# JanBeh/radiorust

Hardware: NVIDIA B200
Metric: complex MS/s via FreqShift->Filter->Downsampler (higher is better)
Workload: dtype f32

## Files before the change

radiorust_b200/csrc/rr_fused.cu:

```cuda
#include <cuda.h>
#include <cuda_runtime.h>

#include <algorithm>
#include <cstdio>
#include <cstdlib>
#include <mutex>

#include "rr_kernels.h"
#include "rr_poly.cuh"
#include "rr_pk.cuh"

namespace rr {

namespace {

constexpr int FK = 512;
constexpr int FRK = 10;
constexpr int T_WARPS = FRK / 2;
constexpr int T_THREADS = 32 * T_WARPS;
constexpr int F_ROWS = 32;
constexpr int PITCH = FRK * 8;
constexpr int STAGE_ROWS = 528;
constexpr int STAGE_BYTES = STAGE_ROWS * PITCH;
constexpr int TW_UNITS = 17;
constexpr int TW_BYTES = 16 * TW_UNITS * 16;
constexpr int YS_STRIDE = FK + 1;

constexpr int kFusedSlots = 6;
constexpr int kFusedSlotFloats = 2560;
__constant__ float4 c_fcoef[kFusedSlots * kFusedSlotFloats / 4];

__device__ __forceinline__ uint32_t s_u32(const void* p) { return (uint32_t)__cvta_generic_to_shared(p); }
__device__ __forceinline__ void mb_init(uint32_t bar, uint32_t count) {
    asm volatile("mbarrier.init.shared::cta.b64 [%0], %1;" ::"r"(bar), "r"(count) : "memory");
}
__device__ __forceinline__ void mb_expect_tx(uint32_t bar, uint32_t bytes) {
    asm volatile("mbarrier.arrive.expect_tx.shared::cta.b64 _, [%0], %1;" ::"r"(bar), "r"(bytes) : "memory");
}
__device__ __forceinline__ void mb_arrive(uint32_t bar) {
    asm volatile("mbarrier.arrive.release.cta.shared::cta.b64 _, [%0];" ::"r"(bar) : "memory");
}
__device__ __forceinline__ void mb_wait(uint32_t bar, uint32_t parity) {
    asm volatile(
        "{\n"
        ".reg .pred p;\n"
        "FWAIT_%=:\n"
        "mbarrier.try_wait.parity.acquire.cta.shared::cta.b64 p, [%0], %1;\n"
        "@p bra FDONE_%=;\n"
        "bra FWAIT_%=;\n"
        "FDONE_%=:\n"
        "}\n" ::"r"(bar),
        "r"(parity)
        : "memory");
}
__device__ __forceinline__ void mb_wait_long(uint32_t bar, uint32_t parity) {
    asm volatile(
        "{\n"
        ".reg .pred p;\n"
        "LWAIT_%=:\n"
        "mbarrier.try_wait.parity.acquire.cta.shared::cta.b64 p, [%0], %1, %2;\n"
        "@p bra LDONE_%=;\n"
        "bra LWAIT_%=;\n"
        "LDONE_%=:\n"
        "}\n" ::"r"(bar),
        "r"(parity), "r"(20000u)
        : "memory");
}
__device__ __forceinline__ pc f_lds(uint32_t addr) {
    pc r;
    asm volatile("ld.shared.v2.f32 {%0, %1}, [%2];" : "=f"(r.x), "=f"(r.y) : "r"(addr));
    return r;
}
__device__ __forceinline__ void f_lds2(uint32_t addr, pc& a, pc& b) {
    asm volatile("ld.shared.v4.f32 {%0, %1, %2, %3}, [%4];" : "=f"(a.x), "=f"(a.y), "=f"(b.x), "=f"(b.y) : "r"(addr));
}
__device__ __forceinline__ void f_sts(uint32_t addr, pc a) {
    asm volatile("st.shared.v2.f32 [%0], {%1, %2};" ::"r"(addr), "f"(a.x), "f"(a.y) : "memory");
}
__device__ __forceinline__ void f_sts2(uint32_t addr, pc a, pc b) {
    asm volatile("st.shared.v4.f32 [%0], {%1, %2, %3, %4};" ::"r"(addr), "f"(a.x), "f"(a.y), "f"(b.x), "f"(b.y) : "memory");
}
__device__ __forceinline__ void f_ldg2(const float4* p, pc& a, pc& b) {
    asm volatile("ld.global.nc.v4.f32 {%0, %1, %2, %3}, [%4];" : "=f"(a.x), "=f"(a.y), "=f"(b.x), "=f"(b.y) : "l"(p));
}

__device__ __forceinline__ pc f_rotation(uint32_t d, uint32_t numer_abs, uint32_t denom, double inv_m, int sign) {
    const uint32_t r = mulmod_fast(numer_abs, d % denom, denom, inv_m);
    double s, c;
    sincospi(2.0 * (double)r / (double)denom, &s, &c);
    return pc((float)c, (float)(sign < 0 ? -s : s));
}

__device__ __forceinline__ void f_pass1_store(pc (&v)[32], uint32_t tw_row, uint32_t xch_wr) {
    pdft_regs<32, +1>(v);
    pc w[3][2];
    f_lds2(tw_row, w[0][0], w[0][1]);
    f_lds2(tw_row + 16, w[1][0], w[1][1]);
#pragma unroll
    for (int m = 0; m < 16; ++m) {
        if (m + 2 < 16) f_lds2(tw_row + (m + 2) * 16, w[(m + 2) % 3][0], w[(m + 2) % 3][1]);
        f_sts(xch_wr + (2 * m) * PITCH, pcmul(v[2 * m], w[m % 3][0]));
        f_sts(xch_wr + (2 * m + 1) * PITCH, pcmul(v[2 * m + 1], w[m % 3][1]));
    }
}

#ifdef RR_FUSED_PROF
#define PROF(...) __VA_ARGS__
__device__ long long g_fused_prof[256 * 16];
#else
#define PROF(...)
#endif

struct FusedGeom {
    int steps, S0, hp, slot_bytes, slot_stride;
};
__host__ __device__ inline FusedGeom fused_geom(int P) {
    FusedGeom g;
    g.steps = P / 2;
    g.S0 = (g.steps + 1) / 2;
    g.hp = 2 * g.S0 + ((g.S0 & 1) ? 0 : 2);
    if (g.hp > P) g.hp = P;
    g.slot_bytes = F_ROWS * g.hp * 8;
    g.slot_stride = (g.slot_bytes + 127) / 128 * 128;
    return g;
}

template <int S_LO, int S_HI, bool HAS_NCO>
__device__ __forceinline__ void f_steps(pc (&acc)[FRK], const float4* __restrict__ xrow, const float4* __restrict__ crow, const float4* cf_base) {
#pragma unroll
    for (int st = S_LO; st < S_HI; ++st) {
        const float4 xv = xrow[st];
        pc x0(xv.x, xv.y), x1(xv.z, xv.w);
        if (HAS_NCO) {
            const float4 cv = crow[st];
            x0 = pcmul(x0, pc(cv.x, cv.y));
            x1 = pcmul(x1, pc(cv.z, cv.w));
        }
        const float4* cf = cf_base + st * 5;
        const float4 a0 = cf[0], a1 = cf[1], a2 = cf[2], a3 = cf[3], a4 = cf[4];
        const float k0[FRK] = {a0.x, a0.y, a0.z, a0.w, a1.x, a1.y, a1.z, a1.w, a2.x, a2.y};
        const float k1[FRK] = {a2.z, a2.w, a3.x, a3.y, a3.z, a3.w, a4.x, a4.y, a4.z, a4.w};
#pragma unroll
        for (int c = 0; c < FRK; ++c) {
            acc[c] = pfma_s(x0, k0[c], acc[c]);
            acc[c] = pfma_s(x1, k1[c], acc[c]);
        }
    }
}

}

template <int FW, int D, int NB, bool HAS_NCO, int PT>
__global__ void __launch_bounds__(T_THREADS + 32 * FW, 1)
k_fused(const __grid_constant__ CUtensorMap tmap, const FusedArgs a, const int n_streams) {
    extern __shared__ __align__(128) unsigned char smem[];
    const int warp = __shfl_sync(0xffffffffu, (int)(threadIdx.x >> 5), 0), lane = threadIdx.x & 31;
    const int P = PT > 0 ? PT : a.P;
    const FusedGeom geo = fused_geom(P);
    const int Lmax = a.Lmax, V = a.V, n_out = a.n_out;
    const int B = (n_out + V - 1) / V;
    const int n_tiles = (B * V + F_ROWS - 1) / F_ROWS;

    const int keep_bytes = ((Lmax * PITCH) + 127) / 128 * 128;
    unsigned char* const p_stage = smem;
    unsigned char* const p_tw = p_stage + 2 * STAGE_BYTES;
    unsigned char* const p_keep = p_tw + TW_BYTES;
    unsigned char* const p_ys = p_keep + keep_bytes;
    unsigned char* const p_ring = p_ys + (((size_t)NB * YS_STRIDE * 8 + 127) / 128 * 128);
    unsigned char* const p_colph = p_ring + (size_t)FW * D * geo.slot_stride;
    unsigned char* const p_bar = p_colph + (((size_t)FW * P * 8 + 127) / 128 * 128);
    const uint32_t bar_full = s_u32(p_bar), bar_empty = bar_full + 16, bar_ring = bar_full + 32;
    const uint32_t left_cnt = bar_ring + FW * D * 8;

    for (int e = threadIdx.x; e < 2 * STAGE_BYTES / 16; e += blockDim.x) reinterpret_cast<float4*>(p_stage)[e] = make_float4(0.f, 0.f, 0.f, 0.f);
    {
        const float2* __restrict__ twK = reinterpret_cast<const float2*>(a.twK);
        for (int e = threadIdx.x; e < FK; e += blockDim.x) {
            const int tr = e >> 5, k1 = e & 31;
            const float2 w = twK[(tr * k1) & (FK - 1)];
            const int off = (tr * TW_UNITS + (k1 >> 1)) * 16 + (k1 & 1) * 8;
            *reinterpret_cast<float2*>(p_tw + off) = w;
        }
    }
    if (threadIdx.x == 0) {
        asm volatile("prefetch.tensormap [%0];" ::"l"(&tmap) : "memory");
        mb_init(bar_full, FW);
        mb_init(bar_full + 8, FW);
        mb_init(bar_empty, T_WARPS);
        mb_init(bar_empty + 8, T_WARPS);
        for (int q = 0; q < FW * D; ++q) mb_init(bar_ring + q * 8, 1);
        asm volatile("st.shared.v2.u32 [%0], {%1, %1};" ::"r"(left_cnt), "r"(0u) : "memory");
        asm volatile("fence.mbarrier_init.release.cluster;" ::: "memory");
    }
    __syncthreads();

    const int n_my = (n_streams - (int)blockIdx.x + (int)gridDim.x - 1) / (int)gridDim.x;
    if (n_my <= 0) return;

    if (warp >= T_WARPS) {
        const int fw = warp - T_WARPS;
        const uint32_t ring_s = s_u32(p_ring) + fw * (D * geo.slot_stride);
        const uint32_t rbar = bar_ring + fw * (D * 8);
        float2* const colph = reinterpret_cast<float2*>(p_colph) + fw * P;
        const int steps = geo.steps, S0 = geo.S0, hp = geo.hp;
        const int half1_col0 = P - hp;
        const int J0 = (int)a.J0;
        const int hist_len = (int)(2 * a.n);
        const int hist_from = (int)a.hist_from;
        const int n_live = (n_out + F_ROWS - 1) / F_ROWS;
        const int rot_step = n_live % FW;
        auto tiles_from = [&](int j0) { return j0 < n_tiles ? (n_tiles - j0 + FW - 1) / FW : 0; };
        const int BV = B * V;
        const int tile_step = FW * F_ROWS;

        int i_so = 0, i_k = 0, i_half = 0, i_slot = 0;
        int i_j0 = fw, i_rot = 0, i_tw = tiles_from(fw);
        auto issue_next = [&]() {
            while (i_so < n_my) {
                if (i_k >= i_tw) {
                    ++i_so;
                    i_k = 0;
                    i_rot += rot_step;
                    if (i_rot >= FW) i_rot -= FW;
                    i_j0 = fw - i_rot + (fw < i_rot ? FW : 0);
                    i_tw = tiles_from(i_j0);
                    continue;
                }
                const int j = i_j0 + i_k * FW, half = i_half, so = i_so;
                i_half ^= 1;
                if (i_half == 0) ++i_k;
                const int rows_ok = min(F_ROWS, n_out - j * F_ROWS);
                if (rows_ok <= 0) continue;
                const int pos0 = j * (F_ROWS * P) - J0;
                const int coff = half ? half1_col0 : 0;
                const int sh = pos0 < 0 ? -1 : F_ROWS - rows_ok;
                if (lane == 0) {
                    mb_expect_tx(rbar + i_slot * 8, (uint32_t)geo.slot_bytes);
                    asm volatile("cp.async.bulk.tensor.3d.shared::cluster.global.mbarrier::complete_tx::bytes [%0], [%1, {%3, %4, %5}], [%2];" ::"r"(
                                     ring_s + i_slot * geo.slot_stride),
                                 "l"(&tmap), "r"(rbar + i_slot * 8), "r"(pos0 + coff - sh * P), "r"(sh), "r"((int)blockIdx.x + so * (int)gridDim.x)
                                 : "memory");
                }
                i_slot = (i_slot + 1 == D) ? 0 : i_slot + 1;
                return;
            }
        };
#pragma unroll 1
        for (int q = 0; q < D; ++q) issue_next();

        PROF(long long pr[8] = {0, 0, 0, 0, 0, 0, 0, 0}; const long long pr_t0 = clock64();)
        int c_slot = 0;
        uint32_t c_phase = 0;
        int gb_acq = -1;
        int gb_arr = -1;
        auto arrive_upto = [&](int gb_done) {
            for (int g2 = gb_arr + 1; g2 <= gb_done; ++g2) {
                while (gb_acq < g2) {
                    ++gb_acq;
                    mb_wait(bar_empty + (uint32_t)(gb_acq & 1) * 8, (uint32_t)(((gb_acq >> 1) & 1) ^ 1));
                }
                __syncwarp();
                if (lane == 0) mb_arrive(bar_full + (uint32_t)(g2 & 1) * 8);
            }
            if (gb_done > gb_arr) gb_arr = gb_done;
        };

        int rot = 0;
#pragma unroll 1
        for (int so = 0; so < n_my; ++so) {
            PROF(const long long pst0 = clock64();)
            const int s = (int)blockIdx.x + so * (int)gridDim.x;
            const int gb0 = so * B;
            const int j0 = fw - rot + (fw < rot ? FW : 0);
            const int tiles_w = tiles_from(j0);
            rot += rot_step;
            if (rot >= FW) rot -= FW;
            uint32_t denom = 1, numer_abs = 0, idx0 = 0;
            int sign = 0;
            float start = 0.f;
            pc rot_tile(1.f, 0.f);
            double inv_denom = 1.0;
            if (HAS_NCO && j0 < n_live) {
                const NcoStream ns = a.nco[s];
                denom = ns.denom;
                numer_abs = ns.numer_abs;
                sign = ns.sign;
                idx0 = ns.idx;
                start = (float)ns.start_phase;
                inv_denom = 1.0 / (double)denom;
                rot_tile = f_rotation((uint32_t)(tile_step * P), numer_abs, denom, inv_denom, sign);
                __syncwarp();
                for (int p = lane; p < P; p += 32) {
                    const pc c = f_rotation((uint32_t)p, numer_abs, denom, inv_denom, sign);
                    colph[p] = make_float2(c.x, c.y);
                }
                __syncwarp();
            }
            const float2* __restrict__ in = reinterpret_cast<const float2*>(a.in) + (long long)s * a.in_stride;
            const float2* __restrict__ hist_end = reinterpret_cast<const float2*>(a.hist2) + ((long long)s + 1) * hist_len;
            float2* __restrict__ hist_o = a.hist_out ? reinterpret_cast<float2*>(a.hist_out) + (long long)s * a.hist_stride : nullptr;
            float4* __restrict__ keep_o = reinterpret_cast<float4*>(reinterpret_cast<float2*>(a.ukeep_out) + (long long)s * a.ukeep_out_stride);
            const float4* cf_base = c_fcoef + a.coef_off4;
            const float4* __restrict__ crow = reinterpret_cast<const float4*>(colph);

            PROF(pr[7] += clock64() - pst0;)
            int blk = (j0 * F_ROWS) / V, off = (j0 * F_ROWS) - blk * V;
            pc rowph(1.f, 0.f);
#pragma unroll 1
            for (int k = 0; k < tiles_w; ++k) {
                const int r0 = (j0 + k * FW) * F_ROWS;
                const int row = r0 + lane;
                const int pos0 = r0 * P - J0;
                pc acc[FRK];
#pragma unroll
                for (int c = 0; c < FRK; ++c) acc[c] = pc(0.f, 0.f);
                PROF(long long pc0 = clock64();)
                if (r0 < n_out) {
                    if (HAS_NCO) {
                        if ((k & 15) == 0) {
                            const long long v = (long long)idx0 + pos0 + (long long)lane * P;
                            long long kk = v - (long long)floor((double)v * inv_denom) * (long long)denom;
                            if (kk < 0) kk += denom;
                            else if (kk >= (long long)denom) kk -= denom;
                            const cx<float> c = nco_phasor<float>(mulmod_fast(numer_abs, (uint32_t)kk, denom, inv_denom), denom, sign, start);
                            rowph = pc(c.x, c.y);
                        } else {
                            rowph = pcmul(rowph, rot_tile);
                        }
                    }
                    const int prow = pos0 + lane * P;
                    const bool to_hist = hist_o != nullptr && pos0 + F_ROWS * P > hist_from;
#pragma unroll 1
                    for (int half = 0; half < 2; ++half) {
                        const uint32_t slot_s = ring_s + c_slot * geo.slot_stride;
                        PROF(long long pw0 = clock64(); pr[0] += pw0 - pc0;)
                        mb_wait(rbar + c_slot * 8, c_phase);
                        PROF(long long pw1 = clock64(); pr[1] += pw1 - pw0;)
                        const int col0 = half ? half1_col0 : 0;
                        if (pos0 < 0) {
                            float2* dst = reinterpret_cast<float2*>(smem + (slot_s - s_u32(smem)));
                            const float r0x = __shfl_sync(0xffffffffu, rowph.x, 0), r0y = __shfl_sync(0xffffffffu, rowph.y, 0);
                            for (int cc = lane; cc < hp; cc += 32) {
                                const int p = col0 + cc;
                                const int pos = pos0 + p;
                                float2 q = make_float2(0.f, 0.f);
                                if (pos >= 0) {
                                    if (pos < (int)a.len) q = __ldg(in + pos);
                                } else if (pos >= -hist_len) {
                                    q = __ldg(hist_end + pos);
                                    if (HAS_NCO) {
                                        const float2 cph = colph[p];
                                        const pc y = pcmulc(pc(q.x, q.y), pcmul(pc(r0x, r0y), pc(cph.x, cph.y)));
                                        q = make_float2(y.x, y.y);
                                    }
                                }
                                dst[cc] = q;
                            }
                            __syncwarp();
                        }
                        const float4* __restrict__ xrow = reinterpret_cast<const float4*>(smem + (slot_s - s_u32(smem)) + lane * (hp * 8) - col0 * 8);
                        if (to_hist) {
                            const int st_lo = half ? S0 : 0, st_hi = half ? steps : S0;
#pragma unroll 2
                            for (int st = st_lo; st < st_hi; ++st) {
                                const float4 xv = xrow[st];
                                pc x0(xv.x, xv.y), x1(xv.z, xv.w);
                                if (HAS_NCO) {
                                    const float4 cv = crow[st];
                                    x0 = pcmul(x0, pc(cv.x, cv.y));
                                    x1 = pcmul(x1, pc(cv.z, cv.w));
                                }
                                const pc y0 = HAS_NCO ? pcmul(x0, rowph) : x0, y1 = HAS_NCO ? pcmul(x1, rowph) : x1;
                                const int jh = prow + 2 * st - hist_from;
                                if (row < n_out && jh >= -1) {
                                    if (jh >= 0) hist_o[jh] = make_float2(y0.x, y0.y);
                                    hist_o[jh + 1] = make_float2(y1.x, y1.y);
                                }
                                const float4* cf = cf_base + st * 5;
                                const float4 a0 = cf[0], a1 = cf[1], a2 = cf[2], a3 = cf[3], a4 = cf[4];
                                const float k0[FRK] = {a0.x, a0.y, a0.z, a0.w, a1.x, a1.y, a1.z, a1.w, a2.x, a2.y};
                                const float k1[FRK] = {a2.z, a2.w, a3.x, a3.y, a3.z, a3.w, a4.x, a4.y, a4.z, a4.w};
#pragma unroll
                                for (int c = 0; c < FRK; ++c) {
                                    acc[c] = pfma_s(x0, k0[c], acc[c]);
                                    acc[c] = pfma_s(x1, k1[c], acc[c]);
                                }
                            }
                        } else if constexpr (PT > 0) {
                            constexpr int STEPS_C = PT / 2, S0_C = (STEPS_C + 1) / 2;
                            if (half == 0) f_steps<0, S0_C, HAS_NCO>(acc, xrow, crow, cf_base);
                            else f_steps<S0_C, STEPS_C, HAS_NCO>(acc, xrow, crow, cf_base);
                        } else {
                            const int st_lo = half ? S0 : 0, st_hi = half ? steps : S0;
#pragma unroll 4
                            for (int st = st_lo; st < st_hi; ++st) {
                                const float4 xv = xrow[st];
                                pc x0(xv.x, xv.y), x1(xv.z, xv.w);
                                if (HAS_NCO) {
                                    const float4 cv = crow[st];
                                    x0 = pcmul(x0, pc(cv.x, cv.y));
                                    x1 = pcmul(x1, pc(cv.z, cv.w));
                                }
                                const float4* cf = cf_base + st * 5;
                                const float4 a0 = cf[0], a1 = cf[1], a2 = cf[2], a3 = cf[3], a4 = cf[4];
                                const float k0[FRK] = {a0.x, a0.y, a0.z, a0.w, a1.x, a1.y, a1.z, a1.w, a2.x, a2.y};
                                const float k1[FRK] = {a2.z, a2.w, a3.x, a3.y, a3.z, a3.w, a4.x, a4.y, a4.z, a4.w};
#pragma unroll
                                for (int c = 0; c < FRK; ++c) {
                                    acc[c] = pfma_s(x0, k0[c], acc[c]);
                                    acc[c] = pfma_s(x1, k1[c], acc[c]);
                                }
                            }
                        }
                        PROF(long long ps1 = clock64(); pr[2] += ps1 - pw1;)
                        asm volatile("fence.proxy.async.shared::cta;" ::: "memory");
                        __syncwarp();
                        PROF(long long ps2 = clock64(); pr[3] += ps2 - ps1;)
                        if (++c_slot == D) {
                            c_slot = 0;
                            c_phase ^= 1u;
                        }
                        issue_next();
                        PROF(pc0 = clock64(); pr[4] += pc0 - ps2;)
                    }
                }
                {
                    const int last_off = min(off + F_ROWS, BV - blk * V) - 1;
                    const int gb_hi = gb0 + blk + (last_off >= V ? 1 : 0);
                    PROF(long long pe0 = clock64(); pr[0] += pe0 - pc0;)
                    while (gb_acq < gb_hi) {
                        ++gb_acq;
                        mb_wait(bar_empty + (uint32_t)(gb_acq & 1) * 8, (uint32_t)(((gb_acq >> 1) & 1) ^ 1));
                    }
                    PROF(pc0 = clock64(); pr[5] += pc0 - pe0;)
                }
                if (row < BV) {
                    int b = blk, o = off + lane;
                    if (o >= V) {
                        o -= V;
                        ++b;
                    }
                    const uint32_t dst = s_u32(p_stage) + (uint32_t)((gb0 + b) & 1) * STAGE_BYTES + (Lmax + o) * PITCH;
                    const bool live = row < n_out;
                    const bool keep = live && row >= n_out - Lmax;
#pragma unroll
                    for (int c = 0; c < FRK; c += 2) {
                        pc y0 = acc[c], y1 = acc[c + 1];
                        if (HAS_NCO) {
                            y0 = pcmul(y0, rowph);
                            y1 = pcmul(y1, rowph);
                        }
                        if (!live) {
                            y0 = pc(0.f, 0.f);
                            y1 = pc(0.f, 0.f);
                        }
                        f_sts2(dst + c * 8, y0, y1);
                        if (keep) keep_o[((row - (n_out - Lmax)) * FRK + c) / 2] = make_float4(y0.x, y0.y, y1.x, y1.y);
                    }
                }
                __syncwarp();
                off += tile_step;
                while (off >= V) {
                    off -= V;
                    ++blk;
                }
                arrive_upto((k + 1 < tiles_w) ? gb0 + min(blk, B) - 1 : gb0 + B - 1);
                PROF(pr[6] += clock64() - pc0;)
            }
            if (tiles_w == 0) arrive_upto(gb0 + B - 1);
        }
        PROF(if (fw == 0 && lane == 0) {
            for (int q = 0; q < 7; ++q) g_fused_prof[blockIdx.x * 16 + q] = pr[q];
            g_fused_prof[blockIdx.x * 16 + 7] = pr[7];
            g_fused_prof[blockIdx.x * 16 + 8] = clock64() - pr_t0;
        })
        return;
    }

    const int tid = threadIdx.x;
    const int t = lane >> 1, gg = lane & 1;
    const int g = 2 * warp + gg;
    auto sync_t = [&]() { asm volatile("bar.sync 1, %0;" ::"n"(T_THREADS) : "memory"); };
    const uint32_t stage0 = s_u32(p_stage);
    const uint32_t tw_row = s_u32(p_tw) + t * (TW_UNITS * 16);
    const uint32_t tile_rd = t * PITCH + g * 8;
    const uint32_t xch_wr = 33 * t * PITCH + g * 8;
    const uint32_t xch_rd = t * PITCH + g * 8;
    const uint32_t keep_s = s_u32(p_keep) + warp * 16;
    float2* const ysave = reinterpret_cast<float2*>(p_ys);
    const float4* __restrict__ gtab = reinterpret_cast<const float4*>(a.gtab);
    const int hist_rows_per_lane = (Lmax + 31) / 32;

    const int n_blocks_total = n_my * B;
    auto copy_kept = [&](int so_k, int gb_k) {
        const uint32_t bytes = (uint32_t)(Lmax * PITCH), bar = bar_full + (uint32_t)(gb_k & 1) * 8;
        const float2* src = reinterpret_cast<const float2*>(a.ukeep_in) + (long long)((int)blockIdx.x + so_k * (int)gridDim.x) * a.ukeep_in_stride;
        asm volatile("fence.proxy.async.shared::cta;" ::: "memory");
        asm volatile("mbarrier.expect_tx.relaxed.cta.shared::cta.b64 [%0], %1;" ::"r"(bar), "r"(bytes) : "memory");
        asm volatile("cp.async.bulk.shared::cluster.global.mbarrier::complete_tx::bytes [%0], [%1], %2, [%3];" ::"r"(stage0 + (uint32_t)(gb_k & 1) * STAGE_BYTES),
                     "l"(src), "r"(bytes), "r"(bar)
                     : "memory");
    };
    if (tid == 0) {
        copy_kept(0, 0);
        if (B == 1 && n_my > 1) copy_kept(1, 1);
    }
    int parked = 0;
    int gb_first = 0;
    int so = 0, b = -1;
    PROF(long long tp[6] = {0, 0, 0, 0, 0, 0}; long long tc = clock64();)

#pragma unroll 1
    for (int gb = 0; gb < n_blocks_total; ++gb) {
        if (++b == B) {
            b = 0;
            ++so;
        }
        const int s = (int)blockIdx.x + so * (int)gridDim.x;
        const uint32_t stg = stage0 + (uint32_t)(gb & 1) * STAGE_BYTES;

        PROF({ long long n_ = clock64(); tp[0] += n_ - tc; tc = n_; })
        mb_wait_long(bar_full + (uint32_t)(gb & 1) * 8, (uint32_t)((gb >> 1) & 1));
        PROF({ long long n_ = clock64(); tp[1] += n_ - tc; tc = n_; })
#pragma unroll
        for (int q = 0; q < 12; ++q) {
            const int r = lane + 32 * q;
            if (q < hist_rows_per_lane && r < Lmax) {
                float4 nx;
                asm volatile("ld.shared.v4.f32 {%0, %1, %2, %3}, [%4];" : "=f"(nx.x), "=f"(nx.y), "=f"(nx.z), "=f"(nx.w) : "r"(stg + (V + r) * PITCH + warp * 16));
                if (b != 0) {
                    float4 h;
                    asm volatile("ld.shared.v4.f32 {%0, %1, %2, %3}, [%4];" : "=f"(h.x), "=f"(h.y), "=f"(h.z), "=f"(h.w) : "r"(keep_s + r * PITCH));
                    asm volatile("st.shared.v4.f32 [%0], {%1, %2, %3, %4};" ::"r"(stg + r * PITCH + warp * 16), "f"(h.x), "f"(h.y), "f"(h.z), "f"(h.w) : "memory");
                }
                asm volatile("st.shared.v4.f32 [%0], {%1, %2, %3, %4};" ::"r"(keep_s + r * PITCH), "f"(nx.x), "f"(nx.y), "f"(nx.z), "f"(nx.w) : "memory");
            }
        }
        if (b == 0 && n_out < Lmax) {
            float4* __restrict__ kout = reinterpret_cast<float4*>(reinterpret_cast<float2*>(a.ukeep_out) + (long long)s * a.ukeep_out_stride);
#pragma unroll 1
            for (int r = n_out + lane; r < Lmax; r += 32) {
                float4 h;
                asm volatile("ld.shared.v4.f32 {%0, %1, %2, %3}, [%4];" : "=f"(h.x), "=f"(h.y), "=f"(h.z), "=f"(h.w) : "r"(stg + r * PITCH + warp * 16));
                kout[((long long)(r - n_out) * FRK) / 2 + warp] = h;
            }
        }
        if (lane == 0) asm volatile("st.shared.v4.f32 [%0], {%1, %1, %1, %1};" ::"r"(stg + (FK - 1) * PITCH + warp * 16), "f"(0.f) : "memory");
        __syncwarp();

        pc acc[32];
        {
            pc v[32];
            const uint32_t src = stg + tile_rd;
#pragma unroll
            for (int m = 0; m < 32; ++m) v[m] = f_lds(src + m * (16 * PITCH));
            __syncwarp();
            f_pass1_store(v, tw_row, stg + xch_wr);
        }
        {
            const float4* gp = gtab + tid;
            pc h[16];
#pragma unroll
            for (int jj = 0; jj < 8; ++jj) f_ldg2(gp + jj * T_THREADS, h[2 * jj], h[2 * jj + 1]);
            __syncwarp();
#pragma unroll
            for (int which = 0; which < 2; ++which) {
                pc x[16];
#pragma unroll
                for (int tr = 0; tr < 16; ++tr) x[tr] = f_lds(stg + xch_rd + (33 * tr + 16 * which) * PITCH);
                pdft_regs<16, +1>(x);
#pragma unroll
                for (int k = 0; k < 16; ++k) acc[which * 16 + k] = pcmul(x[k], h[k]);
                if (which == 0) {
#pragma unroll
                    for (int jj = 0; jj < 8; ++jj) f_ldg2(gp + (8 + jj) * T_THREADS, h[2 * jj], h[2 * jj + 1]);
                }
            }
        }
        PROF({ long long n_ = clock64(); tp[2] += n_ - tc; tc = n_; })
        __syncwarp();
#pragma unroll
        for (int j = 0; j < 32; ++j) f_sts(stg + xch_rd + (16 * j) * PITCH, acc[j]);
        sync_t();
        if (parked == 0) gb_first = gb;
        {
            float2* ys = ysave + parked * YS_STRIDE;
            for (int o = tid; o < FK; o += T_THREADS) {
                const uint32_t src = stg + o * PITCH;
                pc sum(0.f, 0.f);
#pragma unroll
                for (int w = 0; w < T_WARPS; ++w) {
                    pc u0, u1;
                    f_lds2(src + w * 16, u0, u1);
                    sum = sum + u0;
                    sum = sum + u1;
                }
                const int j = o >> 4, tt = o & 15;
                ys[tt + 16 * (j >> 4) + 32 * (j & 15)] = make_float2(sum.x, sum.y);
            }
        }
        ++parked;
        PROF({ long long n_ = clock64(); tp[3] += n_ - tc; tc = n_; })

        if (parked == NB || gb + 1 == n_blocks_total) {
            sync_t();
#pragma unroll 1
            for (int j0 = 0; j0 < parked; j0 += FRK) {
                if (j0 + 2 * warp >= parked) continue;
                const int job = j0 + g;
                const bool active = job < parked;
                pc v[32];
                const float2* ys = ysave + (active ? job : 0) * YS_STRIDE;
#pragma unroll
                for (int i1 = 0; i1 < 32; ++i1) {
                    const float2 q = ys[t + 16 * i1];
                    v[i1] = active ? pc(q.x, -q.y) : pc(0.f, 0.f);
                }
                f_pass1_store(v, tw_row, stg + xch_wr);
                __syncwarp();
                const int gj = gb_first + (active ? job : 0);
                const int so_j = gj / B, b_j = gj - so_j * B;
                const int s_j = (int)blockIdx.x + so_j * (int)gridDim.x;
                float2* __restrict__ out = reinterpret_cast<float2*>(a.out) + (long long)s_j * a.out_stride;
                float2* __restrict__ out2 = a.out2 ? reinterpret_cast<float2*>(a.out2) + (long long)s_j * a.out2_stride : nullptr;
#pragma unroll
                for (int which = 0; which < 2; ++which) {
                    pc x[16];
#pragma unroll
                    for (int tr = 0; tr < 16; ++tr) x[tr] = f_lds(stg + xch_rd + (33 * tr + 16 * which) * PITCH);
                    pdft_regs<16, +1>(x);
                    if (active) {
#pragma unroll
                        for (int k2 = 0; k2 < 16; ++k2) {
                            const int i = t + 16 * which + 32 * k2;
                            if (i >= Lmax && i < Lmax + V) {
                                const long long o = (long long)b_j * V + (i - Lmax);
                                if (o < n_out) {
                                    float2* dst = (out2 != nullptr && o >= a.out_split) ? out2 + (o - a.out_split) : out + o;
                                    *dst = make_float2(x[k2].x, -x[k2].y);
                                }
                            }
                        }
                    }
                }
                __syncwarp();
            }
            parked = 0;
            sync_t();
        }
        PROF({ long long n_ = clock64(); tp[4] += n_ - tc; tc = n_; })
        __syncwarp();
        if (lane == 0) {
            uint32_t left;
            asm volatile("atom.acq_rel.cta.shared::cta.add.u32 %0, [%1], 1;" : "=r"(left) : "r"(left_cnt + (uint32_t)(gb & 1) * 4) : "memory");
            if (left % T_WARPS == T_WARPS - 1) {
                int b2 = b + 2, so2 = so;
                while (b2 >= B) {
                    b2 -= B;
                    ++so2;
                }
                if (b2 == 0 && so2 < n_my) copy_kept(so2, gb + 2);
            }
            mb_arrive(bar_empty + (uint32_t)(gb & 1) * 8);
        }
    }
    PROF(if (tid == 0) for (int q = 0; q < 5; ++q) g_fused_prof[blockIdx.x * 16 + 9 + q] = tp[q];)
}

namespace {

using EncodeFn = CUresult (*)(CUtensorMap*, CUtensorMapDataType, cuuint32_t, void*, const cuuint64_t*, const cuuint64_t*, const cuuint32_t*,
                              const cuuint32_t*, CUtensorMapInterleave, CUtensorMapSwizzle, CUtensorMapL2promotion, CUtensorMapFloatOOBfill);
EncodeFn fused_encode_fn() {
    static EncodeFn fn = nullptr;
    static std::once_flag once;
    std::call_once(once, [] {
        void* p = nullptr;
        cudaDriverEntryPointQueryResult q;
        if (cudaGetDriverEntryPoint("cuTensorMapEncodeTiled", &p, cudaEnableDefault, &q) == cudaSuccess && q == cudaDriverEntryPointSuccess)
            fn = reinterpret_cast<EncodeFn>(p);
    });
    return fn;
}

template <int FW, int D, int NB> size_t fused_smem(int P, int Lmax) {
    const FusedGeom geo = fused_geom(P);
    size_t b = 2 * (size_t)STAGE_BYTES + TW_BYTES;
    b += ((size_t)Lmax * PITCH + 127) / 128 * 128;
    b += ((size_t)NB * YS_STRIDE * 8 + 127) / 128 * 128;
    b += (size_t)FW * D * geo.slot_stride;
    b += ((size_t)FW * P * 8 + 127) / 128 * 128;
    b += 32 + (size_t)FW * D * 8 + 64;
    return b;
}

template <int FW, int D, int NB>
cudaError_t launch_cfg(int n_streams, const FusedArgs& a, const CUtensorMap& tm, int sm_count, cudaStream_t st) {
    const size_t smem = fused_smem<FW, D, NB>(a.P, a.Lmax);
    if (smem > (size_t)227 * 1024) return cudaErrorInvalidConfiguration;
    const int grid = std::min(n_streams, sm_count);
    void (*kern)(const CUtensorMap, const FusedArgs, const int);
    switch (a.P) {
        case 50: kern = a.nco ? k_fused<FW, D, NB, true, 50> : k_fused<FW, D, NB, false, 50>; break;
        case 40: kern = a.nco ? k_fused<FW, D, NB, true, 40> : k_fused<FW, D, NB, false, 40>; break;
        case 20: kern = a.nco ? k_fused<FW, D, NB, true, 20> : k_fused<FW, D, NB, false, 20>; break;
        default: return cudaErrorNotSupported;
    }
    const cudaError_t e = cudaFuncSetAttribute(kern, cudaFuncAttributeMaxDynamicSharedMemorySize, (int)smem);
    if (e != cudaSuccess) return e;
    kern<<<grid, T_THREADS + 32 * FW, smem, st>>>(tm, a, n_streams);
#ifdef RR_FUSED_PROF
    static int calls = 0;
    static int at = std::getenv("RR_FUSED_PROF_CALL") ? std::atoi(std::getenv("RR_FUSED_PROF_CALL")) : 12;
    if (++calls == at) {
        cudaDeviceSynchronize();
        long long h[256 * 16];
        cudaMemcpyFromSymbol(h, g_fused_prof, sizeof h);
        for (int c : {0, 100})
            fprintf(stderr,
                    "cta %d n_out %d F0: tile-head %lld ring-wait %lld steps %lld fence+sync %lld issue %lld empty-wait %lld finalize %lld stream-setup %lld | total %lld"
                    " || T0: pre %lld wait-full %lld fwd+prod %lld sum+park %lld inverse %lld\n",
                    c, a.n_out, h[c * 16], h[c * 16 + 1], h[c * 16 + 2], h[c * 16 + 3], h[c * 16 + 4], h[c * 16 + 5], h[c * 16 + 6], h[c * 16 + 7], h[c * 16 + 8], h[c * 16 + 9],
                    h[c * 16 + 10], h[c * 16 + 11], h[c * 16 + 12], h[c * 16 + 13]);
    }
#endif
    return cudaGetLastError();
}

}

int fused_coef_slots() { return kFusedSlots; }

bool fused_supported(int rank_pad, long long P, int Lmax) {
    if (rank_pad != FRK || !(P == 50 || P == 40 || P == 20) || fused_encode_fn() == nullptr) return false;
    if (Lmax < 1 || FK - 1 - Lmax < 128 || Lmax > 383) return false;
    if ((P / 2) * 2 * FRK > kFusedSlotFloats) return false;
    return fused_smem<7, 2, 5>((int)P, Lmax) <= (size_t)227 * 1024;
}

cudaError_t fused_upload_coef(int slot, const float* acoef, int P, cudaStream_t st) {
    if (slot < 0 || slot >= kFusedSlots) return cudaErrorInvalidValue;
    const size_t n = (size_t)(P / 2) * 2 * FRK;
    if (n > (size_t)kFusedSlotFloats) return cudaErrorInvalidValue;
    return cudaMemcpyToSymbolAsync(c_fcoef, acoef, n * sizeof(float), (size_t)slot * kFusedSlotFloats * sizeof(float), cudaMemcpyHostToDevice, st);
}

cudaError_t launch_fused(int n_streams, const FusedArgs& a0, int sm_count, cudaStream_t st) {
    EncodeFn enc = fused_encode_fn();
    if (!enc) return cudaErrorNotSupported;
    FusedArgs a = a0;
    a.coef_off4 = a.coef_slot * (kFusedSlotFloats / 4);
    if ((uintptr_t)a.ukeep_in % 16 != 0 || (n_streams > 1 && a.ukeep_in_stride % 2 != 0)) return cudaErrorInvalidValue;
    const FusedGeom geo = fused_geom(a.P);
    CUtensorMap tm;
    const cuuint64_t dims[3] = {(cuuint64_t)a.len, (cuuint64_t)F_ROWS, (cuuint64_t)n_streams};
    const cuuint64_t sstride = n_streams > 1 ? (cuuint64_t)a.in_stride * 8 : (((cuuint64_t)a.len * 8 + 15) / 16) * 16;
    const cuuint64_t strides[2] = {(cuuint64_t)a.P * 8, sstride};
    const cuuint32_t box[3] = {(cuuint32_t)geo.hp, (cuuint32_t)F_ROWS, 1};
    const cuuint32_t estr[3] = {1, 1, 1};
    const CUresult r = enc(&tm, CU_TENSOR_MAP_DATA_TYPE_UINT64, 3, const_cast<void*>(a.in), dims, strides, box, estr, CU_TENSOR_MAP_INTERLEAVE_NONE,
                           CU_TENSOR_MAP_SWIZZLE_NONE, CU_TENSOR_MAP_L2_PROMOTION_L2_128B, CU_TENSOR_MAP_FLOAT_OOB_FILL_NONE);
    if (r != CUDA_SUCCESS) return cudaErrorInvalidValue;
    static int cfg = -1;
    if (cfg < 0) {
        cfg = 0;
        if (const char* e = std::getenv("RR_FUSED_CFG")) cfg = std::atoi(e);
    }
    switch (cfg) {
        case 1: return launch_cfg<6, 2, 8>(n_streams, a, tm, sm_count, st);
        default: return launch_cfg<7, 2, 5>(n_streams, a, tm, sm_count, st);
    }
}

}
```

Measured before the change: 529,900.

## Process multiple row groups per filter warp with K column boxes

Generalizes the filter warps so each lane handles R rows (R=2 by default for long outputs), sharing coefficient and column-phasor loads across rows. Each input tile is also split into K column boxes (4 by default) rather than two halves, which keeps ring slots small while tiles get taller. The tensor map is now built per configuration, and the code falls back to R=1, K=2 for short outputs or when shared memory would overflow. The goal is to amortize coefficient loads and per-tile overhead over more rows, at the cost of higher register pressure (20 accumulators per lane) and more barrier and TMA round trips per tile.

Measured after the change: 419,000, median of 6. 20.9% lower.

```diff
diff --git a/radiorust_b200/csrc/rr_fused.cu b/radiorust_b200/csrc/rr_fused.cu
--- a/radiorust_b200/csrc/rr_fused.cu
+++ b/radiorust_b200/csrc/rr_fused.cu
@@ -112,54 +112,68 @@
 #endif
 
 struct FusedGeom {
-    int steps, S0, hp, slot_bytes, slot_stride;
+    int rows, steps, SB, hp, slot_bytes, slot_stride;
 };
-__host__ __device__ inline FusedGeom fused_geom(int P) {
-    FusedGeom g;
+__host__ __device__ constexpr FusedGeom fused_geom(int P, int R, int K) {
+    FusedGeom g{};
+    g.rows = F_ROWS * R;
     g.steps = P / 2;
-    g.S0 = (g.steps + 1) / 2;
-    g.hp = 2 * g.S0 + ((g.S0 & 1) ? 0 : 2);
+    g.SB = (g.steps + K - 1) / K;
+    g.hp = 2 * g.SB + ((g.SB & 1) ? 0 : 2);
     if (g.hp > P) g.hp = P;
-    g.slot_bytes = F_ROWS * g.hp * 8;
+    g.slot_bytes = g.rows * g.hp * 8;
     g.slot_stride = (g.slot_bytes + 127) / 128 * 128;
     return g;
 }
-
-template <int S_LO, int S_HI, bool HAS_NCO>
-__device__ __forceinline__ void f_steps(pc (&acc)[FRK], const float4* __restrict__ xrow, const float4* __restrict__ crow, const float4* cf_base) {
+__host__ __device__ constexpr int fused_box_col0(const FusedGeom& g, int P, int k) { return 2 * k * g.SB < P - g.hp ? 2 * k * g.SB : P - g.hp; }
+
+template <int R, int ROW_F4, int S_LO, int S_HI, bool HAS_NCO>
+__device__ __forceinline__ void f_steps(pc (&acc)[R][FRK], const float4* __restrict__ xrow, const float4* __restrict__ crow, const float4* cf_base) {
 #pragma unroll
     for (int st = S_LO; st < S_HI; ++st) {
-        const float4 xv = xrow[st];
-        pc x0(xv.x, xv.y), x1(xv.z, xv.w);
-        if (HAS_NCO) {
-            const float4 cv = crow[st];
-            x0 = pcmul(x0, pc(cv.x, cv.y));
-            x1 = pcmul(x1, pc(cv.z, cv.w));
-        }
+        float4 cv;
+        if (HAS_NCO) cv = crow[st];
         const float4* cf = cf_base + st * 5;
         const float4 a0 = cf[0], a1 = cf[1], a2 = cf[2], a3 = cf[3], a4 = cf[4];
         const float k0[FRK] = {a0.x, a0.y, a0.z, a0.w, a1.x, a1.y, a1.z, a1.w, a2.x, a2.y};
         const float k1[FRK] = {a2.z, a2.w, a3.x, a3.y, a3.z, a3.w, a4.x, a4.y, a4.z, a4.w};
 #pragma unroll
-        for (int c = 0; c < FRK; ++c) {
-            acc[c] = pfma_s(x0, k0[c], acc[c]);
-            acc[c] = pfma_s(x1, k1[c], acc[c]);
-        }
-    }
-}
-
-}
-
-template <int FW, int D, int NB, bool HAS_NCO, int PT>
+        for (int i = 0; i < R; ++i) {
+            const float4 xv = xrow[i * ROW_F4 + st];
+            pc x0(xv.x, xv.y), x1(xv.z, xv.w);
+            if (HAS_NCO) {
+                x0 = pcmul(x0, pc(cv.x, cv.y));
+                x1 = pcmul(x1, pc(cv.z, cv.w));
+            }
+#pragma unroll
+            for (int c = 0; c < FRK; ++c) {
+                acc[i][c] = pfma_s(x0, k0[c], acc[i][c]);
+                acc[i][c] = pfma_s(x1, k1[c], acc[i][c]);
+            }
+        }
+    }
+}
+
+template <int R, int ROW_F4, int SB, int STEPS, int KB, int K, bool HAS_NCO>
+__device__ __forceinline__ void f_box_steps(int kb, pc (&acc)[R][FRK], const float4* __restrict__ xrow, const float4* __restrict__ crow, const float4* cf_base) {
+    constexpr int HI = (KB + 1) * SB < STEPS ? (KB + 1) * SB : STEPS;
+    if (kb == KB) f_steps<R, ROW_F4, KB * SB, HI, HAS_NCO>(acc, xrow, crow, cf_base);
+    else if constexpr (KB + 1 < K) f_box_steps<R, ROW_F4, SB, STEPS, KB + 1, K, HAS_NCO>(kb, acc, xrow, crow, cf_base);
+}
+
+}
+
+template <int FW, int D, int NB, int R, int K, bool HAS_NCO, int PT>
 __global__ void __launch_bounds__(T_THREADS + 32 * FW, 1)
 k_fused(const __grid_constant__ CUtensorMap tmap, const FusedArgs a, const int n_streams) {
     extern __shared__ __align__(128) unsigned char smem[];
     const int warp = __shfl_sync(0xffffffffu, (int)(threadIdx.x >> 5), 0), lane = threadIdx.x & 31;
-    const int P = PT > 0 ? PT : a.P;
-    const FusedGeom geo = fused_geom(P);
+    constexpr int P = PT;
+    constexpr FusedGeom geo = fused_geom(P, R, K);
+    constexpr int ROWS = geo.rows;
     const int Lmax = a.Lmax, V = a.V, n_out = a.n_out;
     const int B = (n_out + V - 1) / V;
-    const int n_tiles = (B * V + F_ROWS - 1) / F_ROWS;
+    const int n_tiles = (B * V + ROWS - 1) / ROWS;
 
     const int keep_bytes = ((Lmax * PITCH) + 127) / 128 * 128;
     unsigned char* const p_stage = smem;
@@ -202,18 +216,17 @@
         const uint32_t ring_s = s_u32(p_ring) + fw * (D * geo.slot_stride);
         const uint32_t rbar = bar_ring + fw * (D * 8);
         float2* const colph = reinterpret_cast<float2*>(p_colph) + fw * P;
-        const int steps = geo.steps, S0 = geo.S0, hp = geo.hp;
-        const int half1_col0 = P - hp;
+        constexpr int steps = geo.steps, SB = geo.SB, hp = geo.hp;
         const int J0 = (int)a.J0;
         const int hist_len = (int)(2 * a.n);
         const int hist_from = (int)a.hist_from;
-        const int n_live = (n_out + F_ROWS - 1) / F_ROWS;
+        const int n_live = (n_out + ROWS - 1) / ROWS;
         const int rot_step = n_live % FW;
         auto tiles_from = [&](int j0) { return j0 < n_tiles ? (n_tiles - j0 + FW - 1) / FW : 0; };
         const int BV = B * V;
-        const int tile_step = FW * F_ROWS;
-
-        int i_so = 0, i_k = 0, i_half = 0, i_slot = 0;
+        constexpr int tile_step = FW * ROWS;
+
+        int i_so = 0, i_k = 0, i_box = 0, i_slot = 0;
         int i_j0 = fw, i_rot = 0, i_tw = tiles_from(fw);
         auto issue_next = [&]() {
             while (i_so < n_my) {
@@ -226,14 +239,16 @@
                     i_tw = tiles_from(i_j0);
                     continue;
                 }
-                const int j = i_j0 + i_k * FW, half = i_half, so = i_so;
-                i_half ^= 1;
-                if (i_half == 0) ++i_k;
-                const int rows_ok = min(F_ROWS, n_out - j * F_ROWS);
+                const int j = i_j0 + i_k * FW, box = i_box, so = i_so;
+                if (++i_box == K) {
+                    i_box = 0;
+                    ++i_k;
+                }
+                const int rows_ok = min(ROWS, n_out - j * ROWS);
                 if (rows_ok <= 0) continue;
-                const int pos0 = j * (F_ROWS * P) - J0;
-                const int coff = half ? half1_col0 : 0;
-                const int sh = pos0 < 0 ? -1 : F_ROWS - rows_ok;
+                const int pos0 = j * (ROWS * P) - J0;
+                const int coff = fused_box_col0(geo, P, box);
+                const int sh = pos0 < 0 ? -1 : ROWS - rows_ok;
                 if (lane == 0) {
                     mb_expect_tx(rbar + i_slot * 8, (uint32_t)geo.slot_bytes);
                     asm volatile("cp.async.bulk.tensor.3d.shared::cluster.global.mbarrier::complete_tx::bytes [%0], [%1, {%3, %4, %5}], [%2];" ::"r"(
@@ -304,42 +319,49 @@
             const float4* __restrict__ crow = reinterpret_cast<const float4*>(colph);
 
             PROF(pr[7] += clock64() - pst0;)
-            int blk = (j0 * F_ROWS) / V, off = (j0 * F_ROWS) - blk * V;
-            pc rowph(1.f, 0.f);
+            int blk = (j0 * ROWS) / V, off = (j0 * ROWS) - blk * V;
+            pc rowph[R];
+#pragma unroll
+            for (int i = 0; i < R; ++i) rowph[i] = pc(1.f, 0.f);
 #pragma unroll 1
             for (int k = 0; k < tiles_w; ++k) {
-                const int r0 = (j0 + k * FW) * F_ROWS;
-                const int row = r0 + lane;
+                const int r0 = (j0 + k * FW) * ROWS;
                 const int pos0 = r0 * P - J0;
-                pc acc[FRK];
-#pragma unroll
-                for (int c = 0; c < FRK; ++c) acc[c] = pc(0.f, 0.f);
+                pc acc[R][FRK];
+#pragma unroll
+                for (int i = 0; i < R; ++i)
+#pragma unroll
+                    for (int c = 0; c < FRK; ++c) acc[i][c] = pc(0.f, 0.f);
                 PROF(long long pc0 = clock64();)
                 if (r0 < n_out) {
                     if (HAS_NCO) {
-                        if ((k & 15) == 0) {
-                            const long long v = (long long)idx0 + pos0 + (long long)lane * P;
-                            long long kk = v - (long long)floor((double)v * inv_denom) * (long long)denom;
-                            if (kk < 0) kk += denom;
-                            else if (kk >= (long long)denom) kk -= denom;
-                            const cx<float> c = nco_phasor<float>(mulmod_fast(numer_abs, (uint32_t)kk, denom, inv_denom), denom, sign, start);
-                            rowph = pc(c.x, c.y);
+                        if ((k & (16 / R - 1)) == 0) {
+#pragma unroll
+                            for (int i = 0; i < R; ++i) {
+                                const long long v = (long long)idx0 + pos0 + (long long)(lane + 32 * i) * P;
+                                long long kk = v - (long long)floor((double)v * inv_denom) * (long long)denom;
+                                if (kk < 0) kk += denom;
+                                else if (kk >= (long long)denom) kk -= denom;
+                                const cx<float> c = nco_phasor<float>(mulmod_fast(numer_abs, (uint32_t)kk, denom, inv_denom), denom, sign, start);
+                                rowph[i] = pc(c.x, c.y);
+                            }
                         } else {
-                            rowph = pcmul(rowph, rot_tile);
+#pragma unroll
+                            for (int i = 0; i < R; ++i) rowph[i] = pcmul(rowph[i], rot_tile);
                         }
                     }
                     const int prow = pos0 + lane * P;
-                    const bool to_hist = hist_o != nullptr && pos0 + F_ROWS * P > hist_from;
+                    const bool to_hist = hist_o != nullptr && pos0 + ROWS * P > hist_from;
 #pragma unroll 1
-                    for (int half = 0; half < 2; ++half) {
+                    for (int box = 0; box < K; ++box) {
                         const uint32_t slot_s = ring_s + c_slot * geo.slot_stride;
                         PROF(long long pw0 = clock64(); pr[0] += pw0 - pc0;)
                         mb_wait(rbar + c_slot * 8, c_phase);
                         PROF(long long pw1 = clock64(); pr[1] += pw1 - pw0;)
-                        const int col0 = half ? half1_col0 : 0;
+                        const int col0 = fused_box_col0(geo, P, box);
                         if (pos0 < 0) {
                             float2* dst = reinterpret_cast<float2*>(smem + (slot_s - s_u32(smem)));
-                            const float r0x = __shfl_sync(0xffffffffu, rowph.x, 0), r0y = __shfl_sync(0xffffffffu, rowph.y, 0);
+                            const float r0x = __shfl_sync(0xffffffffu, rowph[0].x, 0), r0y = __shfl_sync(0xffffffffu, rowph[0].y, 0);
                             for (int cc = lane; cc < hp; cc += 32) {
                                 const int p = col0 + cc;
                                 const int pos = pos0 + p;
@@ -358,59 +380,41 @@
                             }
                             __syncwarp();
                         }
+                        constexpr int ROW_F4 = 32 * hp / 2;
                         const float4* __restrict__ xrow = reinterpret_cast<const float4*>(smem + (slot_s - s_u32(smem)) + lane * (hp * 8) - col0 * 8);
                         if (to_hist) {
-                            const int st_lo = half ? S0 : 0, st_hi = half ? steps : S0;
-#pragma unroll 2
+                            const int st_lo = box * SB, st_hi = min(st_lo + SB, steps);
+#pragma unroll 1
                             for (int st = st_lo; st < st_hi; ++st) {
-                                const float4 xv = xrow[st];
-                                pc x0(xv.x, xv.y), x1(xv.z, xv.w);
-                                if (HAS_NCO) {
-                                    const float4 cv = crow[st];
-                                    x0 = pcmul(x0, pc(cv.x, cv.y));
-                                    x1 = pcmul(x1, pc(cv.z, cv.w));
-                                }
-                                const pc y0 = HAS_NCO ? pcmul(x0, rowph) : x0, y1 = HAS_NCO ? pcmul(x1, rowph) : x1;
-                                const int jh = prow + 2 * st - hist_from;
-                                if (row < n_out && jh >= -1) {
-                                    if (jh >= 0) hist_o[jh] = make_float2(y0.x, y0.y);
-                                    hist_o[jh + 1] = make_float2(y1.x, y1.y);
-                                }
+                                float4 cv;
+                                if (HAS_NCO) cv = crow[st];
                                 const float4* cf = cf_base + st * 5;
                                 const float4 a0 = cf[0], a1 = cf[1], a2 = cf[2], a3 = cf[3], a4 = cf[4];
                                 const float k0[FRK] = {a0.x, a0.y, a0.z, a0.w, a1.x, a1.y, a1.z, a1.w, a2.x, a2.y};
                                 const float k1[FRK] = {a2.z, a2.w, a3.x, a3.y, a3.z, a3.w, a4.x, a4.y, a4.z, a4.w};
 #pragma unroll
-                                for (int c = 0; c < FRK; ++c) {
-                                    acc[c] = pfma_s(x0, k0[c], acc[c]);
-                                    acc[c] = pfma_s(x1, k1[c], acc[c]);
+                                for (int i = 0; i < R; ++i) {
+                                    const float4 xv = xrow[i * ROW_F4 + st];
+                                    pc x0(xv.x, xv.y), x1(xv.z, xv.w);
+                                    if (HAS_NCO) {
+                                        x0 = pcmul(x0, pc(cv.x, cv.y));
+                                        x1 = pcmul(x1, pc(cv.z, cv.w));
+                                    }
+                                    const pc y0 = HAS_NCO ? pcmul(x0, rowph[i]) : x0, y1 = HAS_NCO ? pcmul(x1, rowph[i]) : x1;
+                                    const int jh = prow + 32 * i * P + 2 * st - hist_from;
+                                    if (r0 + 32 * i + lane < n_out && jh >= -1) {
+                                        if (jh >= 0) hist_o[jh] = make_float2(y0.x, y0.y);
+                                        hist_o[jh + 1] = make_float2(y1.x, y1.y);
+                                    }
+#pragma unroll
+                                    for (int c = 0; c < FRK; ++c) {
+                                        acc[i][c] = pfma_s(x0, k0[c], acc[i][c]);
+                                        acc[i][c] = pfma_s(x1, k1[c], acc[i][c]);
+                                    }
                                 }
                             }
-                        } else if constexpr (PT > 0) {
-                            constexpr int STEPS_C = PT / 2, S0_C = (STEPS_C + 1) / 2;
-                            if (half == 0) f_steps<0, S0_C, HAS_NCO>(acc, xrow, crow, cf_base);
-                            else f_steps<S0_C, STEPS_C, HAS_NCO>(acc, xrow, crow, cf_base);
                         } else {
-                            const int st_lo = half ? S0 : 0, st_hi = half ? steps : S0;
-#pragma unroll 4
-                            for (int st = st_lo; st < st_hi; ++st) {
-                                const float4 xv = xrow[st];
-                                pc x0(xv.x, xv.y), x1(xv.z, xv.w);
-                                if (HAS_NCO) {
-                                    const float4 cv = crow[st];
-                                    x0 = pcmul(x0, pc(cv.x, cv.y));
-                                    x1 = pcmul(x1, pc(cv.z, cv.w));
-                                }
-                                const float4* cf = cf_base + st * 5;
-                                const float4 a0 = cf[0], a1 = cf[1], a2 = cf[2], a3 = cf[3], a4 = cf[4];
-                                const float k0[FRK] = {a0.x, a0.y, a0.z, a0.w, a1.x, a1.y, a1.z, a1.w, a2.x, a2.y};
-                                const float k1[FRK] = {a2.z, a2.w, a3.x, a3.y, a3.z, a3.w, a4.x, a4.y, a4.z, a4.w};
-#pragma unroll
-                                for (int c = 0; c < FRK; ++c) {
-                                    acc[c] = pfma_s(x0, k0[c], acc[c]);
-                                    acc[c] = pfma_s(x1, k1[c], acc[c]);
-                                }
-                            }
+                            f_box_steps<R, ROW_F4, SB, steps, 0, K, HAS_NCO>(box, acc, xrow, crow, cf_base);
                         }
                         PROF(long long ps1 = clock64(); pr[2] += ps1 - pw1;)
                         asm volatile("fence.proxy.async.shared::cta;" ::: "memory");
@@ -425,7 +429,7 @@
                     }
                 }
                 {
-                    const int last_off = min(off + F_ROWS, BV - blk * V) - 1;
+                    const int last_off = min(off + ROWS, BV - blk * V) - 1;
                     const int gb_hi = gb0 + blk + (last_off >= V ? 1 : 0);
                     PROF(long long pe0 = clock64(); pr[0] += pe0 - pc0;)
                     while (gb_acq < gb_hi) {
@@ -434,28 +438,32 @@
                     }
                     PROF(pc0 = clock64(); pr[5] += pc0 - pe0;)
                 }
-                if (row < BV) {
-                    int b = blk, o = off + lane;
-                    if (o >= V) {
-                        o -= V;
-                        ++b;
-                    }
-                    const uint32_t dst = s_u32(p_stage) + (uint32_t)((gb0 + b) & 1) * STAGE_BYTES + (Lmax + o) * PITCH;
-                    const bool live = row < n_out;
-                    const bool keep = live && row >= n_out - Lmax;
-#pragma unroll
-                    for (int c = 0; c < FRK; c += 2) {
-                        pc y0 = acc[c], y1 = acc[c + 1];
-                        if (HAS_NCO) {
-                            y0 = pcmul(y0, rowph);
-                            y1 = pcmul(y1, rowph);
+#pragma unroll
+                for (int i = 0; i < R; ++i) {
+                    const int row = r0 + 32 * i + lane;
+                    if (row < BV) {
+                        int b = blk, o = off + 32 * i + lane;
+                        if (o >= V) {
+                            o -= V;
+                            ++b;
                         }
-                        if (!live) {
-                            y0 = pc(0.f, 0.f);
-                            y1 = pc(0.f, 0.f);
+                        const uint32_t dst = s_u32(p_stage) + (uint32_t)((gb0 + b) & 1) * STAGE_BYTES + (Lmax + o) * PITCH;
+                        const bool live = row < n_out;
+                        const bool keep = live && row >= n_out - Lmax;
+#pragma unroll
+                        for (int c = 0; c < FRK; c += 2) {
+                            pc y0 = acc[i][c], y1 = acc[i][c + 1];
+                            if (HAS_NCO) {
+                                y0 = pcmul(y0, rowph[i]);
+                                y1 = pcmul(y1, rowph[i]);
+                            }
+                            if (!live) {
+                                y0 = pc(0.f, 0.f);
+                                y1 = pc(0.f, 0.f);
+                            }
+                            f_sts2(dst + c * 8, y0, y1);
+                            if (keep) keep_o[((row - (n_out - Lmax)) * FRK + c) / 2] = make_float4(y0.x, y0.y, y1.x, y1.y);
                         }
-                        f_sts2(dst + c * 8, y0, y1);
-                        if (keep) keep_o[((row - (n_out - Lmax)) * FRK + c) / 2] = make_float4(y0.x, y0.y, y1.x, y1.y);
                     }
                 }
                 __syncwarp();
@@ -683,8 +691,8 @@
     return fn;
 }
 
-template <int FW, int D, int NB> size_t fused_smem(int P, int Lmax) {
-    const FusedGeom geo = fused_geom(P);
+template <int FW, int D, int NB, int R, int K> size_t fused_smem(int P, int Lmax) {
+    const FusedGeom geo = fused_geom(P, R, K);
     size_t b = 2 * (size_t)STAGE_BYTES + TW_BYTES;
     b += ((size_t)Lmax * PITCH + 127) / 128 * 128;
     b += ((size_t)NB * YS_STRIDE * 8 + 127) / 128 * 128;
@@ -693,17 +701,29 @@
     b += 32 + (size_t)FW * D * 8 + 64;
     return b;
 }
-
-template <int FW, int D, int NB>
-cudaError_t launch_cfg(int n_streams, const FusedArgs& a, const CUtensorMap& tm, int sm_count, cudaStream_t st) {
-    const size_t smem = fused_smem<FW, D, NB>(a.P, a.Lmax);
-    if (smem > (size_t)227 * 1024) return cudaErrorInvalidConfiguration;
+constexpr size_t kFusedSmemMax = (size_t)227 * 1024;
+constexpr int kFusedR2MinRows = 256;
+
+template <int FW, int D, int NB, int R, int K>
+cudaError_t launch_cfg(int n_streams, const FusedArgs& a, EncodeFn enc, int sm_count, cudaStream_t st) {
+    const size_t smem = fused_smem<FW, D, NB, R, K>(a.P, a.Lmax);
+    if (smem > kFusedSmemMax) return cudaErrorInvalidConfiguration;
+    const FusedGeom geo = fused_geom(a.P, R, K);
+    CUtensorMap tm;
+    const cuuint64_t dims[3] = {(cuuint64_t)a.len, (cuuint64_t)geo.rows, (cuuint64_t)n_streams};
+    const cuuint64_t sstride = n_streams > 1 ? (cuuint64_t)a.in_stride * 8 : (((cuuint64_t)a.len * 8 + 15) / 16) * 16;
+    const cuuint64_t strides[2] = {(cuuint64_t)a.P * 8, sstride};
+    const cuuint32_t box[3] = {(cuuint32_t)geo.hp, (cuuint32_t)geo.rows, 1};
+    const cuuint32_t estr[3] = {1, 1, 1};
+    const CUresult r = enc(&tm, CU_TENSOR_MAP_DATA_TYPE_UINT64, 3, const_cast<void*>(a.in), dims, strides, box, estr, CU_TENSOR_MAP_INTERLEAVE_NONE,
+                           CU_TENSOR_MAP_SWIZZLE_NONE, CU_TENSOR_MAP_L2_PROMOTION_L2_128B, CU_TENSOR_MAP_FLOAT_OOB_FILL_NONE);
+    if (r != CUDA_SUCCESS) return cudaErrorInvalidValue;
     const int grid = std::min(n_streams, sm_count);
     void (*kern)(const CUtensorMap, const FusedArgs, const int);
     switch (a.P) {
-        case 50: kern = a.nco ? k_fused<FW, D, NB, true, 50> : k_fused<FW, D, NB, false, 50>; break;
-        case 40: kern = a.nco ? k_fused<FW, D, NB, true, 40> : k_fused<FW, D, NB, false, 40>; break;
-        case 20: kern = a.nco ? k_fused<FW, D, NB, true, 20> : k_fused<FW, D, NB, false, 20>; break;
+        case 50: kern = a.nco ? k_fused<FW, D, NB, R, K, true, 50> : k_fused<FW, D, NB, R, K, false, 50>; break;
+        case 40: kern = a.nco ? k_fused<FW, D, NB, R, K, true, 40> : k_fused<FW, D, NB, R, K, false, 40>; break;
+        case 20: kern = a.nco ? k_fused<FW, D, NB, R, K, true, 20> : k_fused<FW, D, NB, R, K, false, 20>; break;
         default: return cudaErrorNotSupported;
     }
     const cudaError_t e = cudaFuncSetAttribute(kern, cudaFuncAttributeMaxDynamicSharedMemorySize, (int)smem);
@@ -716,6 +736,7 @@
         cudaDeviceSynchronize();
         long long h[256 * 16];
         cudaMemcpyFromSymbol(h, g_fused_prof, sizeof h);
+        fprintf(stderr, "k_fused<FW %d, R %d, K %d>\n", FW, R, K);
         for (int c : {0, 100})
             fprintf(stderr,
                     "cta %d n_out %d F0: tile-head %lld ring-wait %lld steps %lld fence+sync %lld issue %lld empty-wait %lld finalize %lld stream-setup %lld | total %lld"
@@ -735,7 +756,7 @@
     if (rank_pad != FRK || !(P == 50 || P == 40 || P == 20) || fused_encode_fn() == nullptr) return false;
     if (Lmax < 1 || FK - 1 - Lmax < 128 || Lmax > 383) return false;
     if ((P / 2) * 2 * FRK > kFusedSlotFloats) return false;
-    return fused_smem<7, 2, 5>((int)P, Lmax) <= (size_t)227 * 1024;
+    return fused_smem<7, 2, 5, 1, 2>((int)P, Lmax) <= kFusedSmemMax;
 }
 
 cudaError_t fused_upload_coef(int slot, const float* acoef, int P, cudaStream_t st) {
@@ -751,25 +772,23 @@
     FusedArgs a = a0;
     a.coef_off4 = a.coef_slot * (kFusedSlotFloats / 4);
     if ((uintptr_t)a.ukeep_in % 16 != 0 || (n_streams > 1 && a.ukeep_in_stride % 2 != 0)) return cudaErrorInvalidValue;
-    const FusedGeom geo = fused_geom(a.P);
-    CUtensorMap tm;
-    const cuuint64_t dims[3] = {(cuuint64_t)a.len, (cuuint64_t)F_ROWS, (cuuint64_t)n_streams};
-    const cuuint64_t sstride = n_streams > 1 ? (cuuint64_t)a.in_stride * 8 : (((cuuint64_t)a.len * 8 + 15) / 16) * 16;
-    const cuuint64_t strides[2] = {(cuuint64_t)a.P * 8, sstride};
-    const cuuint32_t box[3] = {(cuuint32_t)geo.hp, (cuuint32_t)F_ROWS, 1};
-    const cuuint32_t estr[3] = {1, 1, 1};
-    const CUresult r = enc(&tm, CU_TENSOR_MAP_DATA_TYPE_UINT64, 3, const_cast<void*>(a.in), dims, strides, box, estr, CU_TENSOR_MAP_INTERLEAVE_NONE,
-                           CU_TENSOR_MAP_SWIZZLE_NONE, CU_TENSOR_MAP_L2_PROMOTION_L2_128B, CU_TENSOR_MAP_FLOAT_OOB_FILL_NONE);
-    if (r != CUDA_SUCCESS) return cudaErrorInvalidValue;
     static int cfg = -1;
     if (cfg < 0) {
         cfg = 0;
         if (const char* e = std::getenv("RR_FUSED_CFG")) cfg = std::atoi(e);
     }
-    switch (cfg) {
-        case 1: return launch_cfg<6, 2, 8>(n_streams, a, tm, sm_count, st);
-        default: return launch_cfg<7, 2, 5>(n_streams, a, tm, sm_count, st);
-    }
-}
-
-}
+    if (a.n_out >= kFusedR2MinRows) {
+        cudaError_t e = cudaErrorInvalidConfiguration;
+        switch (cfg) {
+            case 1: e = launch_cfg<6, 2, 8, 1, 2>(n_streams, a, enc, sm_count, st); break;
+            case 2: e = launch_cfg<7, 2, 5, 2, 4>(n_streams, a, enc, sm_count, st); break;
+            case 3: e = launch_cfg<4, 2, 5, 2, 2>(n_streams, a, enc, sm_count, st); break;
+            case 4: break;
+            default: e = launch_cfg<7, 2, 5, 2, 4>(n_streams, a, enc, sm_count, st); break;
+        }
+        if (e != cudaErrorInvalidConfiguration) return e;
+    }
+    return launch_cfg<7, 2, 5, 1, 2>(n_streams, a, enc, sm_count, st);
+}
+
+}
```
